# ducha-aiki/mods

Hardware: AMD Instinct MI355X
Metric: image-pairs/sec (1024x768, HessAff+RootSIFT over the affine view ladder, MFMA FGINN match, LO-RANSAC H) (higher is better)
Workload: dtype f32 (detect/describe) + u8 on the int8 matrix cores (distance matrix)

## Files before the change

mods_amd/__init__.py:

```python
import ctypes as C
import os
import subprocess

import numpy as np

_HERE = os.path.dirname(os.path.abspath(__file__))
LIB_PATH = os.environ.get("MODSX_LIB", os.path.join(_HERE, "libmodsx.so"))

KEYPOINT = np.dtype([("x", "f8"), ("y", "f8"), ("a11", "f8"), ("a12", "f8"), ("a21", "f8"), ("a22", "f8"),
                     ("s", "f8"), ("response", "f8"), ("octave_number", "i4"), ("pyramid_scale", "f8"),
                     ("sub_type", "i4")], align=True)
REGION = np.dtype([("img_id", "i4"), ("img_reproj_id", "i4"), ("id", "i4"), ("parent_id", "i4"), ("type", "i4"),
                   ("det_kp", KEYPOINT), ("reproj_kp", KEYPOINT)], align=True)
SSKP = np.dtype([("octave", "i4"), ("level", "i4"), ("r0", "i4"), ("c0", "i4"), ("r", "i4"), ("c", "i4"),
                 ("type", "i4"), ("pad", "i4"), ("b0", "f4"), ("b1", "f4"), ("b2", "f4"), ("val", "f4"),
                 ("x", "f4"), ("y", "f4"), ("s", "f4"), ("pixelDistance", "f4")], align=True)
TENT = np.dtype([("q", "i4"), ("t0", "i4"), ("tj", "i4"), ("t1", "i4"), ("d1", "f8"), ("d2", "f8"),
                 ("d2by2ndcl", "f8"), ("ratio", "f8")], align=True)


class HessAffParams(C.Structure):
    _fields_ = [("threshold", C.c_float), ("mode", C.c_int), ("reg_number", C.c_int),
                ("rel_threshold", C.c_float), ("rel_reg_number", C.c_float), ("numberOfScales", C.c_int),
                ("initialSigma", C.c_float), ("edgeEigenValueRatio", C.c_double), ("border", C.c_int),
                ("maxIterations", C.c_int), ("convergenceThreshold", C.c_float), ("smmWindowSize", C.c_int),
                ("affInitialSigma", C.c_float), ("doBaumberg", C.c_int), ("detectorType", C.c_int)]


class MserParams(C.Structure):
    _fields_ = [("min_size", C.c_int), ("max_area", C.c_double), ("min_margin", C.c_double), ("relative", C.c_int),
                ("mode", C.c_int), ("reg_number", C.c_int), ("rel_threshold", C.c_float), ("rel_reg_number", C.c_float)]


class PairParams(C.Structure):
    _fields_ = [("det", HessAffParams),
                ("ori_mrSize", C.c_double), ("ori_patchSize", C.c_int), ("ori_maxAngles", C.c_int),
                ("ori_threshold", C.c_double),
                ("desc_mrSize", C.c_double), ("desc_patchSize", C.c_int), ("desc_photoNorm", C.c_int),
                ("desc_type", C.c_int), ("desc_maxBinValue", C.c_double),
                ("match_ratio", C.c_double), ("contradDist", C.c_double), ("nn", C.c_int),
                ("duplicateDist", C.c_double),
                ("err_threshold", C.c_double), ("confidence", C.c_double), ("max_samples", C.c_int),
                ("localOptimization", C.c_int), ("HLAFCoef", C.c_double), ("doSymmCheck", C.c_int),
                ("ransac_seed", C.c_uint), ("useF", C.c_int), ("LAFCoef", C.c_double), ("errorType", C.c_int),
                ("detector", C.c_int), ("mser", MserParams),
                ("n_desc", C.c_int), ("desc_types", C.c_int * 4), ("desc_ratios", C.c_double * 4)]


class View(C.Structure):
    _fields_ = [("zoom", C.c_double), ("tilt", C.c_double), ("phi", C.c_double), ("InitSigma", C.c_double),
                ("doBlur", C.c_int)]


def make_view(tilt=1.0, phi=0.0, zoom=1.0, init_sigma=0.5, do_blur=1):
    v = View()
    v.zoom, v.tilt, v.phi, v.InitSigma, v.doBlur = zoom, tilt, phi, init_sigma, do_blur
    return v


def _view_array(views):
    arr = (View * len(views))()
    for i, v in enumerate(views):
        arr[i].zoom, arr[i].tilt, arr[i].phi, arr[i].InitSigma, arr[i].doBlur = v.zoom, v.tilt, v.phi, v.InitSigma, v.doBlur
    return arr


class LadderStep(C.Structure):
    _fields_ = [("views", C.c_void_p), ("nviews", C.c_int), ("match_ratio", C.c_double), ("detector", C.c_int),
                ("n_desc", C.c_int), ("desc_types", C.c_int * 4), ("desc_ratios", C.c_double * 4)]


class PairResult(C.Structure):
    _fields_ = [("n_regions1", C.c_int), ("n_regions2", C.c_int), ("n_tentatives", C.c_int), ("n_unique", C.c_int),
                ("n_ransac_inliers", C.c_int), ("n_verified", C.c_int), ("ransac_samples", C.c_int),
                ("ransac_lo", C.c_int), ("H", C.c_double * 9), ("tentatives", C.c_void_p),
                ("ransac_inlier", C.c_void_p), ("verified", C.c_void_p)]


EXPORTS = ["modsx_version", "modsx_last_error", "modsx_free", "modsx_create", "modsx_destroy", "modsx_synchronize",
           "modsx_default_hessaff_params", "modsx_default_pair_params", "modsx_image_upload", "modsx_image_update",
           "modsx_image_wrap_device", "modsx_image_free", "modsx_image_download", "modsx_detect_affine_keypoints",
           "modsx_detect_scalespace", "modsx_octave_levels", "modsx_gaussian_blur", "modsx_resize_half", "modsx_response",
           "modsx_detect_affine_regions", "modsx_detect_orientation", "modsx_reproject_regions", "modsx_reproject_regions_touch_boundary",
           "modsx_describe_regions", "modsx_match_fginn", "modsx_duplicate_filtering", "modsx_ransac_h",
           "modsx_loransac_h", "modsx_ransac_h_errtype", "modsx_loransac_h_errtype", "modsx_ransac_f", "modsx_loransac_f", "modsx_match_pair", "modsx_match_pairs", "modsx_match_pairs_views", "modsx_pair_result_release",
           "modsx_set_vs_pars", "modsx_synth_view", "modsx_detect_describe_views", "modsx_match_fginn_device",
           "modsx_match_pair_views", "modsx_match_ladder", "modsx_save_regions", "modsx_load_regions", "modsx_default_mser_params", "modsx_detect_msers", "modsx_detect_msers_u8", "modsx_last_timings", "modsx_profile",
           "modsx_kernel_stats", "modsx_last_batch_verify", "modsx_comm_unique_id", "modsx_comm_create", "modsx_comm_destroy", "modsx_comm_info",
           "modsx_view_block_order", "modsx_detect_describe_views_sharded", "modsx_match_fginn_sharded",
           "modsx_match_pair_views_sharded", "modsx_match_pairs_views_sharded", "modsx_match_ladder_sharded", "modsx_comm_loopback_id", "modsx_comm_set_lanes",
           "modsx_comm_attach", "modsx_comm_lane_done", "modsx_comm_reset_lanes", "modsx_comm_set_timeout", "modsx_comm_stats",
           "modsx_shard_block_bytes", "modsx_shard_block_pack", "modsx_shard_blocks_unpack", "modsx_shard_device_pack",
           "modsx_shard_device_unpack", "modsx_verify_device_stats", "modsx_verify_device_timing", "modsx_comm_set_exchange",
           "modsx_shard_owner_plan", "modsx_db_create", "modsx_db_free", "modsx_db_rows", "modsx_db_nearest",
           "modsx_match_fginn_db", "modsx_match_fginn_db_device", "modsx_set_fginn_db"]
EXPORTS_DEGENSAC = ["exp_ransacHcustom", "exp_ransacFcustom", "HDs", "HDsi", "HDsidx", "HDsSym", "HDsiSym", "HDsSymidx",
                    "HDsSymMax", "HDsiSymMax", "HDsSymidxMax", "FDs", "FDsSym", "exFDs", "exFDsSym",
                    "modsx_ransac_set_seed"]

SHARD_ROW_REGION, SHARD_ROW_KP = 0, 1
EXCHANGE_ALL_GATHER, EXCHANGE_OWNER = 0, 1
KP_FIELDS = ("x", "y", "a11", "a12", "a21", "a22", "s")
KERNEL_CLASSES = ["blur_hess", "hessian", "resize", "nms_localize", "baumberg", "orientation", "patch_sample",
                  "blur_rows", "describe", "match_fginn", "gray", "warp_affine", "view_blur", "blur_cols", "match_sweep1", "match_db"]


def build(force=False):
    src = os.path.join(_HERE, "csrc")
    srcs = [os.path.join(src, f) for f in os.listdir(src) if f.endswith((".hip", ".cpp", ".hpp"))]
    srcs.append(os.path.join(_HERE, "..", "include", "modsx.h"))
    stale = (not os.path.exists(LIB_PATH)) or any(os.path.getmtime(s) > os.path.getmtime(LIB_PATH) for s in srcs)
    if force or stale:
        subprocess.check_call(["make", "-C", src, "-j8"], stdout=subprocess.DEVNULL)
    return LIB_PATH


_lib = None


def lib():
    global _lib
    if _lib is None:
        if not os.path.exists(LIB_PATH):
            raise RuntimeError("libmodsx.so is not built; run __graft_entry__.build() (needs hipcc)")
        L = C.CDLL(LIB_PATH)
        L.modsx_last_error.restype = C.c_char_p
        L.modsx_create.restype = C.c_void_p
        L.modsx_create.argtypes = [C.c_int]
        L.modsx_comm_create.restype = C.c_void_p
        L.modsx_comm_create.argtypes = [C.c_void_p, C.c_void_p, C.c_int, C.c_int]
        L.modsx_comm_destroy.argtypes = [C.c_void_p]
        L.modsx_comm_info.argtypes = [C.c_void_p] + [C.c_void_p] * 5
        L.modsx_comm_loopback_id.argtypes = [C.c_void_p, C.c_int]
        L.modsx_comm_set_lanes.argtypes = [C.c_void_p, C.c_int]
        L.modsx_comm_attach.argtypes = [C.c_void_p, C.c_void_p, C.c_int]
        L.modsx_comm_lane_done.argtypes = [C.c_void_p, C.c_int]
        L.modsx_comm_reset_lanes.argtypes = [C.c_void_p]
        L.modsx_comm_set_timeout.argtypes = [C.c_void_p, C.c_int]
        L.modsx_comm_stats.argtypes = [C.c_void_p, C.c_void_p, C.c_int]
        L.modsx_destroy.argtypes = [C.c_void_p]
        L.modsx_free.argtypes = [C.c_void_p]
        L.modsx_image_upload.restype = C.c_void_p
        L.modsx_image_upload.argtypes = [C.c_void_p, C.c_void_p, C.c_int, C.c_int, C.c_int, C.c_int]
        L.modsx_image_update.argtypes = [C.c_void_p, C.c_void_p, C.c_void_p, C.c_int, C.c_int, C.c_int, C.c_int]
        L.modsx_debug_last_batch_verify_each.argtypes = [C.c_void_p, C.c_int]
        L.modsx_image_wrap_device.restype = C.c_void_p
        L.modsx_image_wrap_device.argtypes = [C.c_void_p, C.c_void_p, C.c_int, C.c_int]
        L.modsx_image_free.argtypes = [C.c_void_p, C.c_void_p]
        L.modsx_db_create.restype = C.c_void_p
        L.modsx_db_create.argtypes = [C.c_void_p, C.c_void_p, C.c_long, C.c_int]
        L.modsx_db_free.restype = None
        L.modsx_db_free.argtypes = [C.c_void_p, C.c_void_p]
        L.modsx_db_rows.restype = C.c_long
        L.modsx_db_rows.argtypes = [C.c_void_p]
        L.modsx_db_nearest.argtypes = [C.c_void_p, C.c_void_p, C.c_void_p, C.c_int, C.c_void_p]
        L.modsx_set_fginn_db.argtypes = [C.c_void_p, C.c_void_p]
        L.modsx_synth_view.restype = C.c_void_p
        L.modsx_synth_view.argtypes = [C.c_void_p, C.c_void_p, C.c_void_p, C.c_void_p, C.c_void_p]
        _lib = L
    return _lib


def _err():
    return lib().modsx_last_error().decode()


def _p(a):
    return a.ctypes.data_as(C.c_void_p)


def _check(rc, what):
    if rc < 0:
        raise RuntimeError("%s failed (%d): %s" % (what, rc, _err()))
    return rc


def default_hessaff_params(**kw):
    p = HessAffParams()
    lib().modsx_default_hessaff_params(C.byref(p))
    for k, v in kw.items():
        setattr(p, k, v)
    return p


def default_mser_params(**kw):
    p = MserParams()
    lib().modsx_default_mser_params(C.byref(p))
# ... 685 lines not shown
```

mods_amd/csrc/engine.hip:

```cpp
#include <atomic>
#include <math.h>
#include <stdio.h>
#include <algorithm>
#include <chrono>
#include <map>
#include <unordered_set>
#include <mutex>
#include <dlfcn.h>
#include <string>
#include "engine_api.hpp"

#ifdef MODSX_DUP_BUILD
namespace mx {
int dup_count(int cls) {
  static const long mask = getenv("MODSX_DUP") ? strtol(getenv("MODSX_DUP"), nullptr, 0) : 0;
  return 1 + (int)((mask >> cls) & 1);
}
}
#endif
namespace mx {

static thread_local std::string g_err;
void set_error(const std::string &s) { g_err = s; }
static std::atomic<int> g_busyContexts{0};
// ... 348 lines not shown
  for (int i = 0; i < MAXB; i++) { c->descF[i].release(); c->descU8[i].release(); c->viewImg[i].release(); for (int k = 0; k < 3; k++) c->descU8x[k][i].release(); }
  for (int d = 0; d < 2; d++) for (int t = 0; t < 4; t++) for (int sd = 0; sd < 2; sd++) c->descCls[d][t][sd].release();
  for (int t = 0; t < 4; t++) c->halfDesc[t].release();
  c->candSort.release(); c->candOut.release();
  PinBuf *pins[] = {&c->hCand, &c->hAff, &c->hOri, &c->hDesc, &c->hMisc, &c->hNms, &c->hMatch, &c->hViewTaps, &c->hViewJobs, &c->hMser};
  for (PinBuf *b : pins) b->release();
  hipFree(c->dSmmMask); hipFree(c->dOriMask); hipFree(c->dOriIdx); hipFree(c->dSiftMask); hipFree(c->dSiftMaskIdx); hipFree(c->dAtan); hipFree(c->dOriBinTab); hipFree(c->dSiftOTab); hipFree(c->dSiftBins);
  hipFree(c->dSiftW);
  for (int i = 0; i < 2; i++) hipEventDestroy(c->descEv[i]);
  c->hDescB.release(); c->hRefs.release();
  hipStreamDestroy(c->stream);
  if (c->hFlag) hipHostFree(c->hFlag);
  delete c;
}

static int cv_round(double v) { return (int)lrint(v); }

struct SigmaPlan {
  int levels;
  float sigmaStep;
  float curSigma[8];
  float incSigma[8];
};

static SigmaPlan make_sigma_plan(const modsx_hessaff_params &p) {
  SigmaPlan s;
  s.levels = p.numberOfScales + 2;
  s.sigmaStep = powf(2.0f, 1.0f / (float)p.numberOfScales);
  float cur = p.initialSigma;
  s.curSigma[0] = cur; s.incSigma[0] = 0;
  for (int i = 1; i < s.levels; i++) {
    s.incSigma[i] = cur * sqrtf(s.sigmaStep * s.sigmaStep - 1.0f);
    cur *= s.sigmaStep;
    s.curSigma[i] = cur;
  }
  return s;
}

static int fill_taps(BlurBatch &b, float sigma) {
  int n = blur_ksize(sigma);
  if (n > MAX_TAPS) { set_error("pyramid blur kernel larger than 17 taps is not supported"); return MODSX_ERR_ARG; }
  std::vector<float> k = gaussian_kernel(n, sigma);
  b.n = n;
  for (int i = 0; i < n; i++) b.k[i] = k[i];
  return MODSX_OK;
}

int build_pyramids(modsx_ctx *c, const modsx_image *const *imgs, int n, const modsx_hessaff_params &p,
                   bool singleOctaveFromFirstLevel) {
  if (n <= 0 || n > MAXB) { set_error("batch size"); return MODSX_ERR_ARG; }
  if (p.numberOfScales < 1 || p.numberOfScales > 6) { set_error("numberOfScales"); return MODSX_ERR_ARG; }
  if (p.detectorType != MODSX_DET_HESSIAN && p.detectorType != MODSX_DET_DOG && p.detectorType != MODSX_DET_HARRIS) {
    set_error("detectorType must be Hessian (0), DoG (1) or Harris (2)");
    return MODSX_ERR_ARG;
  }
  const bool hess = p.detectorType == MODSX_DET_HESSIAN;
  const SigmaPlan sp = make_sigma_plan(p);
  const int L = sp.levels;
  const int minSize = 2 * p.border + 2;
  int maxOct = 0;
  for (int i = 0; i < n; i++) {
    Pyramid &py = c->pyr[i];
    py.nOct = 0;
    int rows = imgs[i]->rows, cols = imgs[i]->cols;
    float pd = 1.0f;
    size_t total = 0;
    while (rows > minSize && cols > minSize && py.nOct < 24) {
      Octave &o = py.oct[py.nOct++];
      o.rows = rows; o.cols = cols; o.pixelDistance = pd;
      total += (size_t)2 * L * rows * cols;
      pd *= 2.0;
      rows = cv_round(rows * 0.5); cols = cv_round(cols * 0.5);
      if (singleOctaveFromFirstLevel) break;
    }
    if (!py.store.ensure(total * sizeof(float) + 64)) return MODSX_ERR_NOMEM;
    float *ptr = (float *)py.store.p;
    for (int o = 0; o < py.nOct; o++) {
      size_t npx = (size_t)py.oct[o].rows * py.oct[o].cols;
      for (int l = 0; l < L; l++) { py.oct[o].blur[l] = ptr; ptr += npx; }
      for (int l = 0; l < L; l++) { py.oct[o].resp[l] = ptr; ptr += npx; }
    }
    maxOct = std::max(maxOct, py.nOct);
  }
  hipStream_t s = c->stream;
  for (int o = 0; o < maxOct; o++) {
    BlurBatch bb;
    memset(&bb, 0, sizeof bb);
    int nj = 0, mr = 0, mc = 0;
    if (o == 0) {
      const float curSigma0 = 0.5f;
      const bool preBlur = !singleOctaveFromFirstLevel && p.initialSigma > curSigma0;
      if (preBlur) {
        float sigma = sqrtf(p.initialSigma * p.initialSigma - curSigma0 * curSigma0);
        int rc = fill_taps(bb, sigma);
        if (rc) return rc;
      }
      for (int i = 0; i < n; i++) {
        if (c->pyr[i].nOct <= 0) continue;
        Octave &oc = c->pyr[i].oct[0];
        BlurJob &j = bb.j[nj++];
        j.src = imgs[i]->d; j.blur = oc.blur[0]; j.resp = hess ? oc.resp[0] : nullptr; j.rows = oc.rows; j.cols = oc.cols;
        j.norm = sp.curSigma[0] * sp.curSigma[0];
        mr = std::max(mr, oc.rows); mc = std::max(mc, oc.cols);
        if (!preBlur) {
          MX_HIP(hipMemcpyAsync(oc.blur[0], imgs[i]->d, (size_t)oc.rows * oc.cols * 4, hipMemcpyDeviceToDevice, s));
          j.src = oc.blur[0];
        }
      }
      double px = 0;
      for (int q = 0; q < nj; q++) px += (double)bb.j[q].rows * bb.j[q].cols;
      if (nj) {
        if (preBlur) { ProfScope ps(c, K_BLUR_HESS, px * 12); launch_blur_hess(s, bb, nj, mr, mc); }
        else if (hess) { ProfScope ps(c, K_HESSIAN, px * 8); launch_hessian(s, bb, nj, mr, mc); }
      }
    } else {
      ResizeBatch rb;
      memset(&rb, 0, sizeof rb);
      for (int i = 0; i < n; i++) {
        if (c->pyr[i].nOct <= o) continue;
        Octave &pv = c->pyr[i].oct[o - 1], &oc = c->pyr[i].oct[o];
        ResizeJob &r = rb.j[nj];
        r.src = pv.blur[p.numberOfScales]; r.dst = oc.blur[0];
        r.srows = pv.rows; r.scols = pv.cols; r.drows = oc.rows; r.dcols = oc.cols;
        r.resp = hess ? oc.resp[0] : nullptr; r.norm = sp.curSigma[0] * sp.curSigma[0];
        BlurJob &j = bb.j[nj++];
        j.src = oc.blur[0]; j.blur = nullptr; j.resp = oc.resp[0]; j.rows = oc.rows; j.cols = oc.cols;
        j.norm = sp.curSigma[0] * sp.curSigma[0];
        mr = std::max(mr, oc.rows); mc = std::max(mc, oc.cols);
      }
      if (nj) {
        double spx = 0, dpx = 0;
        for (int q = 0; q < nj; q++) { spx += (double)rb.j[q].srows * rb.j[q].scols; dpx += (double)rb.j[q].drows * rb.j[q].dcols; }
        { ProfScope ps(c, K_RESIZE, (spx + dpx) * 4 + dpx * 4); launch_resize_half(s, rb, nj, mr, mc); }
      }
    }
    if (!nj) continue;
    for (int l = 1; l < L; l++) {
      BlurBatch b2;
      memset(&b2, 0, sizeof b2);
      int rc = fill_taps(b2, sp.incSigma[l]);
      if (rc) return rc;
      int k = 0;
      for (int i = 0; i < n; i++) {
        if (c->pyr[i].nOct <= o) continue;
        Octave &oc = c->pyr[i].oct[o];
        BlurJob &j = b2.j[k++];
        j.src = oc.blur[l - 1]; j.blur = oc.blur[l]; j.resp = hess ? oc.resp[l] : nullptr; j.rows = oc.rows; j.cols = oc.cols;
        j.norm = sp.curSigma[l] * sp.curSigma[l];
      }
      double px = 0;
      for (int q = 0; q < k; q++) px += (double)b2.j[q].rows * b2.j[q].cols;
      ProfScope ps(c, K_BLUR_HESS, px * 12);
      launch_blur_hess(s, b2, k, mr, mc);
    }
    if (!hess) {
      for (int l = 0; l < L; l++) {
        const float norm = sp.curSigma[l] * sp.curSigma[l];
        const float sigma = p.detectorType == MODSX_DET_DOG ? norm : sqrtf((float)(0.6 * norm));
        const int nt = blur_ksize(sigma);
        if (2 * nt > 2 * 4096) { set_error("response blur kernel too large"); return MODSX_ERR_ARG; }
        if (!c->viewTaps.ensure((size_t)L * 2 * 4100 * 4) || !c->hViewTaps.ensure((size_t)L * 2 * 4100 * 4)) return MODSX_ERR_NOMEM;
        float *dT = (float *)c->viewTaps.p + (size_t)l * 2 * 4100, *hT = (float *)c->hViewTaps.p + (size_t)l * 2 * 4100;
        bool tapsUp = false;
        for (int i = 0; i < n; i++) {
          if (c->pyr[i].nOct <= o) continue;
          Octave &oc = c->pyr[i].oct[o];
          const int rows = oc.rows, cols = oc.cols;
          const size_t npx = (size_t)rows * cols;
          if (!c->scratchA.ensure(npx * 4 * 8)) return MODSX_ERR_NOMEM;
          float *buf = (float *)c->scratchA.p, *tmp = buf, *a = buf + npx, *b = buf + 2 * npx, *cc = buf + 3 * npx;
          float *ba = buf + 4 * npx, *bb2 = buf + 5 * npx, *bc = buf + 6 * npx;
          const int nx = cols == 1 ? 1 : nt, ny = rows == 1 ? 1 : nt;
          if (!tapsUp || nx != nt || ny != nt) {
            std::vector<float> kx = gaussian_kernel(nx, sigma), ky = gaussian_kernel(ny, sigma);
            if (tapsUp) MX_HIP(ctx_sync(c));
            memcpy(hT, kx.data(), nx * 4); memcpy(hT + nx, ky.data(), ny * 4);
            MX_HIP(ctx_copy(c, dT, hT, (size_t)(nx + ny) * 4, hipMemcpyHostToDevice));
            tapsUp = nx == nt && ny == nt;
          }
          auto blur = [&](const float *src, float *dst) {
            if (nt == 1) { MX_HIP(hipMemcpyAsync(dst, src, npx * 4, hipMemcpyDeviceToDevice, s)); return MODSX_OK; }
            launch_blur_pass(s, src, tmp, rows, cols, dT, nx, 0, 1);
            launch_blur_pass(s, tmp, dst, rows, cols, dT + nx, ny, 1, 1);
            return MODSX_OK;
          };
          if (p.detectorType == MODSX_DET_DOG) {
            int rc = blur(oc.blur[l], a);
            if (rc) return rc;
            launch_sub(s, oc.blur[l], a, oc.resp[l], npx);
          } else {
            launch_grad_products(s, oc.blur[l], rows, cols, a, b, cc);
            int rc = blur(a, ba);
            if (!rc) rc = blur(b, bb2);
            if (!rc) rc = blur(cc, bc);
            if (rc) return rc;
            launch_harris_combine(s, ba, bb2, bc, (float)(0.6 * norm), oc.resp[l], npx);
          }
        }
      }
    }
  }
  MX_HIP(hipGetLastError());
  return MODSX_OK;
}

static const unsigned CAND_CAP = 1u << 21;

int detect_scalespace_batch(modsx_ctx *c, const modsx_image *const *imgs, int n, const modsx_hessaff_params &p,
                            std::vector<modsx_sskp> *out) {
  int rc = build_pyramids(c, imgs, n, p, false);
  if (rc) return rc;
  hipStream_t s = c->stream;
  if (!c->cand.ensure((size_t)CAND_CAP * sizeof(Candidate)) || !c->nmsQueue.ensure((size_t)CAND_CAP * 16)) return MODSX_ERR_NOMEM;
  if (!c->counter.ensure((NMS_QUEUES + 1) * 128)) return MODSX_ERR_NOMEM;
  MX_HIP(hipMemsetAsync(c->counter.p, 0, 128 + NMS_QUEUES * 128, s));
  bool queuesClean = true;
  NmsBatch nb;
  memset(&nb, 0, sizeof nb);
  nb.edgeScoreThreshold = (p.edgeEigenValueRatio + 1.0f) * (p.edgeEigenValueRatio + 1.0f) / p.edgeEigenValueRatio;
  float finalTh = p.threshold;
  float posTh = (float)(0.8 * finalTh);
  float negTh = -posTh;
  if (p.detectorType == MODSX_DET_HESSIAN) finalTh = p.threshold * p.threshold;
  if (p.mode != MODSX_FIXED_TH) finalTh = posTh = negTh = 0.0f;
  nb.posTh = posTh; nb.negTh = negTh; nb.finalTh = finalTh; nb.border = p.border; nb.detType = p.detectorType;
  int maxOct = 0;
  for (int i = 0; i < n; i++) maxOct = std::max(maxOct, c->pyr[i].nOct);
  const bool perOctave = p.numberOfScales == 3 && !getenv("MODSX_NMS_PER_LEVEL");
  std::vector<NmsJob> hjobs;
  std::vector<int> hpfx(1, 0), hfirst;
  double px = 0;
  auto flush = [&](bool last) -> int {
    const int nj = (int)hjobs.size();
    if (!nj) return MODSX_OK;
    const int np = (int)hpfx.size() - 1;
    const size_t jobBytes = (size_t)nj * sizeof(NmsJob), pfxBytes = (size_t)(np + 1) * 4, firstBytes = (size_t)std::max<size_t>(1, hfirst.size()) * 4;
    if (!c->nmsJobs.ensure(jobBytes + pfxBytes + firstBytes + 64)) return MODSX_ERR_NOMEM;
    if (!c->hNms.ensure(jobBytes + pfxBytes + firstBytes)) return MODSX_ERR_NOMEM;
    memcpy(c->hNms.p, hjobs.data(), jobBytes);
    memcpy((char *)c->hNms.p + jobBytes, hpfx.data(), pfxBytes);
    if (!hfirst.empty()) memcpy((char *)c->hNms.p + jobBytes + pfxBytes, hfirst.data(), hfirst.size() * 4);
    MX_HIP(ctx_copy(c, c->nmsJobs.p, c->hNms.p, jobBytes + pfxBytes + firstBytes, hipMemcpyHostToDevice));
    if (!c->tileJob.ensure((size_t)hpfx.back() * 4 + 4)) return MODSX_ERR_NOMEM;
    const int *dPfx = (const int *)((char *)c->nmsJobs.p + jobBytes);
    launch_expand_tiles(s, dPfx, np, (int *)c->tileJob.p);
    {
      ProfScope ps(c, K_NMS, px * 12);
      if (!queuesClean) MX_HIP(hipMemsetAsync((unsigned *)c->counter.p + 32, 0, NMS_QUEUES * 128, s));
      queuesClean = false;
      launch_nms(s, nb, (const NmsJob *)c->nmsJobs.p, dPfx, (const int *)c->tileJob.p, nj,
                 hpfx.back(), (int4 *)c->nmsQueue.p, (unsigned *)c->counter.p + 32, CAND_CAP, (Candidate *)c->cand.p,
                 (unsigned *)c->counter.p, CAND_CAP, perOctave ? (const int *)((char *)c->nmsJobs.p + jobBytes + pfxBytes) : nullptr,
                 p.numberOfScales);
    }
    if (!last) MX_HIP(ctx_sync(c));
    hjobs.clear(); hpfx.assign(1, 0); hfirst.clear(); px = 0;
    return MODSX_OK;
  };
  for (int o = 0; o < maxOct; o++)
    for (int i = 0; i < n; i++) {
      if (c->pyr[i].nOct <= o) continue;
      Octave &oc = c->pyr[i].oct[o];
      const int w = oc.cols - 2 * p.border, h = oc.rows - 2 * p.border;
      if (w <= 0 || h <= 0) continue;
      if ((int)hjobs.size() + p.numberOfScales > NMS_MAXJ) { int rcf = flush(false); if (rcf) return rcf; }
      const int tiles = ((w + 63) / 64) * ((h + NMS_TILE_ROWS - 1) / NMS_TILE_ROWS);
      if (perOctave) { hfirst.push_back((int)hjobs.size()); hpfx.push_back(hpfx.back() + tiles); }
      for (int l = 1; l <= p.numberOfScales; l++) {
        NmsJob j;
        j.low = oc.resp[l - 1]; j.cur = oc.resp[l]; j.high = oc.resp[l + 1]; j.blur = oc.blur[l];
        j.rows = oc.rows; j.cols = oc.cols; j.img = i; j.octave = o; j.level = l; j.pad = 0;
        hjobs.push_back(j);
        if (!perOctave) hpfx.push_back(hpfx.back() + tiles);
        px += (double)oc.rows * oc.cols;
      }
    }
  { int rcf = flush(true); if (rcf) return rcf; }
  static const bool deviceOrder = getenv("MODSX_DEVICE_ORDER") != nullptr && atoi(getenv("MODSX_DEVICE_ORDER")) != 0;
  if (deviceOrder) {
    typedef size_t (*temp_fn)(unsigned);
    typedef int (*order_fn)(hipStream_t, const Candidate *, const unsigned *, unsigned, unsigned long long *, unsigned long long *, unsigned *, unsigned *,
                            void *, size_t, unsigned long long *, unsigned *, unsigned, unsigned *, Candidate *, unsigned *);
// ... 1205 lines not shown
```

mods_amd/csrc/engine.hpp:

```cpp
#pragma once
#include <hip/hip_runtime.h>
#include <stdint.h>
#include <stdlib.h>
#include <string.h>
#include <string>
#include <vector>
#include "../../include/modsx.h"
#include "kmath.hpp"

namespace mx {

#ifndef MODSX_MAXB
#define MODSX_MAXB 32
#endif
constexpr int MAXB = MODSX_MAXB;
constexpr int PAIR_GROUP = 4;
constexpr int NMS_MAXJ = 1024;
constexpr int MAX_TAPS = 17;

struct BlurJob {
  const float *src;
  float *blur;
  float *resp;
  int rows, cols;
  float norm;
  int pad;
};
struct BlurBatch {
  int n;
  float k[MAX_TAPS];
  BlurJob j[MAXB];
  int nj;
  int tile0[MAXB + 1];
};
struct ResizeJob {
  const float *src;
  float *dst;
  float *resp;
  int srows, scols, drows, dcols;
  float norm;
  int pad;
};
struct ResizeBatch { ResizeJob j[MAXB]; int nj; int tile0[MAXB + 1]; };
struct NmsJob {
  const float *low, *cur, *high, *blur;
  int rows, cols, img, octave, level, pad;
};
struct NmsBatch {
  float posTh, negTh, finalTh;
  int border;
  double edgeScoreThreshold;
  int detType, pad;
};
struct Candidate {
  int img, octave, level, type;
  int r0, c0, r, c;
  float b0, b1, b2, val;
};

struct AffJob {
  const float *blur;
  int rows, cols;
  float x, y, s, pixelDistance;
};
struct AffOut { float u11, u12, u21, u22; int ok; int iters; };

struct OriJob {
  int img;
  float x, y, a11, a12, a21, a22;
};
constexpr int ORI_MAX_PEAKS = 18;

struct DescJob {
  int img;
  int P;
  int ksize;
  int tapOfs;
  float x, y, a11, a12, a21, a22;
  float i2p;
  int NC;
  int needOfs;
  int coordOfs;
  int touch;
  int outIdx;
  int rows0;
  int ro1;
  unsigned long long scratchOfs;
  unsigned long long rowOfs;
  unsigned long long gridOfs;
};
struct BlurTile {
  unsigned long long srcOfs, dstOfs;
  int P, NC, n, tapOfs, needOfs;
  int job, pad;
  int first, count, lo, span, magic;
};
struct ImgRef { const float *d; int rows, cols, pad; };
struct DescOut { float *f[MAXB]; uint8_t *u8[MAXB]; uint8_t *u8x[3][MAXB]; };

struct WarpJob {
  const float *src;
  float *dst;
  int srows, scols, drows, dcols;
  double M[6];
  float cval;
  int pad;
};

struct ViewJob {
  const float *src;
  float *rot, *tmp, *dst;
  int srows, scols, rrows, rcols, drows, dcols;
  int kx, ky, tapOfs, doBlur;
  int tileA, tileB;
  int tileF, fused;
  int tileG, pad;
  double R[6], W[6];
  double invW[2];
};

struct MatchRow {
  int t0, t1, nless, nbad;
  int tj;
  float dj;
  float d0, d1;
};
static_assert(sizeof(MatchRow) == 32, "match rows are 32 bytes");

struct DevBuf {
  void *p = nullptr;
  size_t cap = 0;
  bool ensure(size_t bytes);
  void release();
};
struct PinBuf {
  void *p = nullptr;
  size_t cap = 0;
  bool ensure(size_t bytes);
  void release();
};

struct Octave {
  int rows, cols;
  float pixelDistance;
  float *blur[8];
  float *resp[8];
};
struct Pyramid {
  int nOct = 0;
  Octave oct[24];
  DevBuf store;
};

void set_error(const std::string &s);
bool gpu_shared();
struct CtxBusy { modsx_ctx *c; explicit CtxBusy(modsx_ctx *c); ~CtxBusy(); CtxBusy(const CtxBusy &) = delete; CtxBusy &operator=(const CtxBusy &) = delete; };
hipError_t ctx_copy(modsx_ctx *c, void *dst, const void *src, size_t bytes, hipMemcpyKind kind);
hipError_t ctx_sync(modsx_ctx *c);
unsigned ctx_mark(modsx_ctx *c);
bool ctx_mark_reached(modsx_ctx *c, unsigned seq);
hipError_t ctx_wait_mark(modsx_ctx *c, unsigned seq);
bool host_wait_runtime();
int host_cpus_per_rank();
#define MX_HIP(expr)                                                                          \
  do {                                                                                        \
    hipError_t e_ = (expr);                                                                   \
    if (e_ != hipSuccess) {                                                                   \
      mx::set_error(std::string(#expr) + ": " + hipGetErrorString(e_));                       \
      return MODSX_ERR_DEVICE;                                                                \
    }                                                                                         \
  } while (0)

std::vector<float> gaussian_kernel(int n, double sigma);
int blur_ksize(float sigma);
void gauss_mask(float *mask, int size);
void circular_gauss_mask(float *mask, int size, float sigma);
const double *atan_lut_host();
inline bool check_borders_host(int w, int h, float ofsx, float ofsy, float a11, float a12, float a21, float a22, int rw, int rh) {
  return check_borders(w, h, ofsx, ofsy, a11, a12, a21, a22, rw, rh);
}
bool invert3(const double *S, double *t);
void rectify(double &a11, double &a12, double &a21, double &a22);

void launch_blur_hess(hipStream_t s, const BlurBatch &b, int nj, int maxRows, int maxCols);
void launch_hessian(hipStream_t s, const BlurBatch &b, int nj, int maxRows, int maxCols);
void launch_resize_half(hipStream_t s, const ResizeBatch &b, int nj, int maxRows, int maxCols);
void launch_nms(hipStream_t s, const NmsBatch &b, const NmsJob *jobs, const int *tilePrefix, const int *tileJob, int nj,
                int nTiles, int4 *queue, unsigned *qcount, unsigned qcap, Candidate *out, unsigned *counter, unsigned cap,
                const int *octFirst = nullptr, int levelsPerOctave = 0);
size_t cand_sort_temp_bytes(unsigned nsort);
int launch_cand_order(hipStream_t s, const Candidate *cand, const unsigned *counter, unsigned nsort, unsigned long long *keys,
                      unsigned long long *keys2, unsigned *idx, unsigned *idx2, void *temp, size_t tempBytes, unsigned long long *tabKey,
                      unsigned *tabRank, unsigned tabSize, unsigned *slotOf, Candidate *out, unsigned *outCount);
constexpr int NMS_QUEUES = 64;
constexpr int NMS_TILE_ROWS = 16;
void launch_gray(hipStream_t s, const void *src, float *dst, size_t n, int channels, int dtype);
void launch_baumberg(hipStream_t s, const AffJob *jobs, AffOut *out, int n, const float *mask, int W, int maxIter,
                     float convTh, float affInitialSigma);
constexpr int ATAN_CASES = 2048 + 64;
constexpr int ORI_NV = 1344;
void launch_orientation(hipStream_t s, const OriJob *jobs, float *out, int n, const ImgRef *imgs,
                        const unsigned short *maskIdx, const float *maskW,
                        const unsigned char *binTab, int doHalf, double th, int maxAngles);
void launch_trunc_u8(hipStream_t s, const float *src, uint8_t *dst, size_t n);
size_t mser_sort_blocks(const int *rows, int n);
void launch_mser_sort(hipStream_t s, const uint8_t *const *u8, const int *rows, const int *cols, const size_t *ordOfs, int n, int *blockHist,
                      int *start, int *order);
void launch_expand_blur_tiles(hipStream_t s, const DescJob *jobs, const int *prefixRows, const int *prefixCols, int nJobs,
                              const int *needTab, BlurTile *tilesRows, BlurTile *tilesCols, float2 *rowStarts);
void launch_sample_rows(hipStream_t s, const DescJob *jobs, const BlurTile *tiles, int nTiles, const ImgRef *imgs, const float *taps,
                        const int *needTab, float *dst, const float2 *rowStarts, float *dstGrid);
void launch_blur_cols(hipStream_t s, const BlurTile *tiles, int nTiles, const float *taps, const int *needTab, const float *src,
                      float *dst);
void launch_expand_tiles(hipStream_t s, const int *prefix, int nJobs, int *tileJob);
void launch_patch_sample(hipStream_t s, const DescJob *jobs, const int *tilePrefix, const int *tileJob, int nTiles,
                         const ImgRef *imgs, float *scratch);
void launch_patch_blur(hipStream_t s, const DescJob *jobs, const int *tilePrefix, const int *tileJob, int nTiles,
                       const float *taps, const int *needTab, const float *src, float *dst, int pass);
void launch_describe(hipStream_t s, const DescJob *jobs, int n, const ImgRef *imgs, const float *grid,
                     const int *needTab, const float *coordTab,
                     const float *mask, const unsigned short *maskIdx, int nmask, const float *oTab, const int *bins,
                     const double *wts, int photoNorm, int descTypes, int nOut, double maxBin, const DescOut &outs);
void launch_warp_affine(hipStream_t s, const WarpJob &jb);
void launch_blur_pass(hipStream_t s, const float *src, float *dst, int rows, int cols, const float *taps, int n, int pass, int border = 0);
void launch_sub(hipStream_t s, const float *a, const float *b, float *o, size_t n);
void launch_grad_products(hipStream_t s, const float *img, int rows, int cols, float *xx, float *yy, float *xy);
void launch_harris_combine(hipStream_t s, const float *bxx, const float *byy, const float *bxy, float sigmasq, float *o, size_t n);
void launch_views_warp(hipStream_t s, const ViewJob *jobs, int n, int tiles, int stage);
void launch_views_blur(hipStream_t s, const ViewJob *jobs, int n, int tiles, const float *taps, int pass);
constexpr int VF_TW = 128, VF_TH = 16, VF_RX = 32, VF_RY = 2;
void launch_views_rotblur(hipStream_t s, const ViewJob *jobs, int n, int tiles, const float *taps, int maxRx, int maxRy);
void launch_views_fused(hipStream_t s, const ViewJob *jobs, int n, int tiles, const float *taps, int maxRx, int maxRy);
size_t match_workspace_bytes(int n1, int n2);
void launch_match(hipStream_t s, const uint8_t *d1, int n1, const uint8_t *d2, int n2, const double *pos2,
                  double sqminratio, double contrDistSq, int nn, MatchRow *rows, void *workspace);
#ifndef MODSX_SR_WIN
#define MODSX_SR_WIN 2400
#define MODSX_FC_ROWS 40
#define MODSX_SR_HALF 1
#define MODSX_SR_WGS 8
#endif
#ifndef MODSX_BLUR_LDS_C
#define MODSX_BLUR_LDS_C 9984
#endif
constexpr int MATCH_NN_MAX = 256;
constexpr int MATCH_MAXB = 4;
void launch_match_batch(hipStream_t s, int nb, const uint8_t *const *d1, const int *n1, const uint8_t *const *d2, const int *n2,
                        const double *const *pos2, double sqminratio, double contrDistSq, int nn, MatchRow *const *rows,
                        void *const *workspace, hipEvent_t *evSweep1 = nullptr);
struct DbGeo { int TEp, TOp; };
struct DbSet {
  DevBuf store;
  const unsigned char *tiles = nullptr;
  const int *hrow = nullptr;
  DbGeo geo = {0, 0};
  long rows = 0;
  int dev = 0;
};
DbGeo db_geo(long n, long nOdd);
size_t db_tiles_bytes(const DbGeo &g);
size_t db_hrow_bytes(const DbGeo &g);
int db_pack_blocks(long n);
void launch_db_pack(hipStream_t s, const uint8_t *raw, long n, const int2 *base, long nOdd, const DbGeo &geo, unsigned char *tiles,
                    int *hrow);
void launch_db_select(hipStream_t s, int nb, const MatchRow *const *rows, const int *n1, int nn, bool allPoints, int *const *sel, int *cnt,
                      int *const *dmin);
void launch_dbnn_min(hipStream_t s, int nb, const uint8_t *const *d1, const int *n1, int *const *sel, int *cnt, int *const *dmin,
                     const DbSet &db);

}

namespace mx {
#ifdef MODSX_DUP_BUILD
int dup_count(int cls);
#define MX_DUP(cls) for (int dupLeft_ = mx::dup_count(cls); dupLeft_ > 0; dupLeft_--)
#else
#define MX_DUP(cls)
#endif
enum KClass { K_BLUR_HESS = 0, K_HESSIAN, K_RESIZE, K_NMS, K_BAUMBERG, K_ORIENT, K_PATCH_SAMPLE, K_BLUR_ROWS, K_DESCRIBE,
              K_MATCH, K_GRAY, K_WARP, K_VIEW_BLUR, K_BLUR_COLS, K_MATCH_SWEEP1, K_MATCH_DB, K_NCLASS };
struct Profiler {
  bool enabled = false;
  std::vector<hipEvent_t> evA, evB;
  std::vector<int> cls;
  size_t used = 0;
  double ms[K_NCLASS] = {0};
  double work[K_NCLASS] = {0};
  long launches[K_NCLASS] = {0};
};
}

struct modsx_db { mx::DbSet set; };

struct modsx_image {
  float *d;
  int rows, cols;
  bool owned;
};

struct modsx_ctx {
  int dev;
  hipStream_t stream;
  mx::Pyramid pyr[mx::MAXB];
  mx::DevBuf candSort, candOut;
  size_t lastSurvivors = 0;
  mx::DevBuf nmsJobs, cand, counter, affJobs, affOut, oriJobs, oriOut, descJobs, tilePrefix, taps, imgRefs, scratchA, scratchB,
      descF[mx::MAXB], descU8[mx::MAXB], descAllF[2], descAllU8[2], descAllU8b[2], descCls[2][4][2], descU8x[3][mx::MAXB], shardLocal, pos2, matchRows, matchWork, dbSel, misc, viewTmp[2], viewTaps, viewJobs, viewImg[mx::MAXB], scratchC, needTab, coordTab, tileJob, blurTiles, nmsQueue, rowStarts;
  mx::ImgRef imgRefsHost[mx::MAXB];
  mx::PinBuf hDescB;
  hipEvent_t descEv[2];
  bool descEvPending[2] = {false, false};
  bool descByEvent[2] = {true, true};
  unsigned descMark[2] = {0, 0};
  unsigned *hFlag = nullptr;
  unsigned flagSeq = 0;
  bool waitRuntime = true;
  mx::PinBuf hCand, hAff, hOri, hDesc, hMisc, hNms, hMatch, hViewTaps, hViewJobs, hMser, hRefs;
  float *dSmmMask = nullptr;
  int smmW = 0;
  std::vector<uint64_t> candKeys, candKeys2, candClaim;
  std::vector<uint32_t> candOrder, candOrder2;
  float *dOriMask = nullptr;
  unsigned short *dOriIdx = nullptr;
  float *dSiftMask = nullptr;
  unsigned short *dSiftMaskIdx = nullptr;
  int nSiftMask = 0;
  double *dAtan = nullptr;
  unsigned char *dOriBinTab = nullptr;
  float *dSiftOTab = nullptr;
  int *dSiftBins = nullptr;
  double *dSiftW = nullptr;
  double timings[6];
  mx::Profiler prof;
  size_t lastCandCount = 0;
  const mx::DbSet *fginnDb = nullptr;
  int busyDepth = 0;
  int shardLane = 0;
  modsx_ctx *peer = nullptr;
  modsx_ctx *half = nullptr;
  mx::DevBuf halfDesc[4];
  void *worker = nullptr;
};
```

mods_amd/csrc/kernels_pyramid.hip:

```cpp
#include "engine.hpp"

namespace mx {

constexpr int TW = 64;
constexpr int TMP_W = TW + 4;

MX_D int find_job(const int *tile0, int nj, int t) {
  int j = 0;
  while (j + 1 < nj && t >= tile0[j + 1]) j++;
  return j;
}

typedef float f2 __attribute__((ext_vector_type(2)));

template <int R, int TH>
__global__ __launch_bounds__(256) void k_blur_hess(BlurBatch batch) {
  constexpr int BLR_H = TH + 4;
  const int ji = find_job(batch.tile0, batch.nj, blockIdx.x);
  const BlurJob jb = batch.j[ji];
  const int rows = jb.rows, cols = jb.cols;
  const int lt = blockIdx.x - batch.tile0[ji], ntx = (cols + TW - 1) / TW;
  const int tx0 = (lt % ntx) * TW, ty0 = (lt / ntx) * TH;
  constexpr int n = 2 * R + 1;
  constexpr int sh = BLR_H + 2 * R, sw = TMP_W + 2 * R;
// ... 76 lines not shown
      if (gy >= 1 && gy < rows - 1 && gx >= 1 && gx < cols - 1) {
        const float v11 = B[-TMP_W - 1], v12 = B[-TMP_W], v13 = B[-TMP_W + 1];
        const float v21 = B[-1], v22 = B[0], v23 = B[1];
        const float v31 = B[TMP_W - 1], v32 = B[TMP_W], v33 = B[TMP_W + 1];
        float Lxx = (v21 - 2 * v22 + v23);
        float Lyy = (v12 - 2 * v22 + v32);
        float Lxy = (v13 - v11 + v31 - v33) / 4.0f;
        o = (Lxx * Lyy - Lxy * Lxy) * norm2;
      }
      jb.resp[gofs] = o;
    }
  }
}

__global__ __launch_bounds__(256) void k_hessian(BlurBatch batch) {
  const int ji = find_job(batch.tile0, batch.nj, blockIdx.x);
  const BlurJob jb = batch.j[ji];
  const int rows = jb.rows, cols = jb.cols;
  const int lt = blockIdx.x - batch.tile0[ji], ntx = (cols + 63) / 64;
  const int gx = (lt % ntx) * 64 + (threadIdx.x & 63), gy = (lt / ntx) * 4 + (threadIdx.x >> 6);
  if (gx >= cols || gy >= rows) return;
  float o = 0.f;
  if (gy >= 1 && gy < rows - 1 && gx >= 1 && gx < cols - 1) {
    const float *B = jb.src + (size_t)gy * cols + gx;
    const float v11 = B[-cols - 1], v12 = B[-cols], v13 = B[-cols + 1];
    const float v21 = B[-1], v22 = B[0], v23 = B[1];
    const float v31 = B[cols - 1], v32 = B[cols], v33 = B[cols + 1];
    float Lxx = (v21 - 2 * v22 + v23);
    float Lyy = (v12 - 2 * v22 + v32);
    float Lxy = (v13 - v11 + v31 - v33) / 4.0f;
    o = (Lxx * Lyy - Lxy * Lxy) * (jb.norm * jb.norm);
  }
  jb.resp[(size_t)gy * cols + gx] = o;
}

MX_D float resize_half_px(const float *src, int sr, int sc, int dx, int dy) {
  const int sy0 = dy * 2, sx0 = dx * 2;
  float out;
  if (sy0 >= sr) out = 0.f;
  else if (sy0 + 2 <= sr && dx < sc / 2) {
    const float *S = src + (size_t)sy0 * sc + sx0;
    float sum = 0.f;
    sum = sum + (((S[0] + S[1]) + S[sc]) + S[sc + 1]);
    out = sum * 0.25f;
  } else {
    float sum = 0.f; int count = 0;
    for (int sy = 0; sy < 2; sy++) {
      if (sy0 + sy >= sr) break;
      for (int sx = 0; sx < 2; sx++) {
        if (sx0 + sx >= sc) break;
        sum += src[(size_t)(sy0 + sy) * sc + sx0 + sx];
        count++;
      }
    }
    out = (sx0 >= sc) ? 0.f : sum / (float)count;
  }
  return out;
}
__global__ __launch_bounds__(256) void k_resize_half(ResizeBatch batch) {
  const int ji = find_job(batch.tile0, batch.nj, blockIdx.x);
  const ResizeJob jb = batch.j[ji];
  const int lt = blockIdx.x - batch.tile0[ji], ntx = (jb.dcols + 63) / 64;
  const int dx = (lt % ntx) * 64 + (threadIdx.x & 63), dy = (lt / ntx) * 4 + (threadIdx.x >> 6);
  if (dx >= jb.dcols || dy >= jb.drows) return;
  const int sr = jb.srows, sc = jb.scols, rows = jb.drows, cols = jb.dcols;
  const float v22 = resize_half_px(jb.src, sr, sc, dx, dy);
  jb.dst[(size_t)dy * cols + dx] = v22;
  if (!jb.resp) return;
  float o = 0.f;
  if (dy >= 1 && dy < rows - 1 && dx >= 1 && dx < cols - 1) {
    const float v11 = resize_half_px(jb.src, sr, sc, dx - 1, dy - 1), v12 = resize_half_px(jb.src, sr, sc, dx, dy - 1),
                v13 = resize_half_px(jb.src, sr, sc, dx + 1, dy - 1);
    const float v21 = resize_half_px(jb.src, sr, sc, dx - 1, dy), v23 = resize_half_px(jb.src, sr, sc, dx + 1, dy);
    const float v31 = resize_half_px(jb.src, sr, sc, dx - 1, dy + 1), v32 = resize_half_px(jb.src, sr, sc, dx, dy + 1),
                v33 = resize_half_px(jb.src, sr, sc, dx + 1, dy + 1);
    float Lxx = (v21 - 2 * v22 + v23);
    float Lyy = (v12 - 2 * v22 + v32);
    float Lxy = (v13 - v11 + v31 - v33) / 4.0f;
    o = (Lxx * Lyy - Lxy * Lxy) * (jb.norm * jb.norm);
  }
  jb.resp[(size_t)dy * cols + dx] = o;
}

MX_D bool is_max9(float val, const float *p, int cols) {
  bool ok = true;
#pragma unroll
  for (int dr = -1; dr <= 1; dr++)
#pragma unroll
    for (int dc = -1; dc <= 1; dc++) ok = ok && !(p[dr * cols + dc] > val);
  return ok;
}
MX_D bool is_min9(float val, const float *p, int cols) {
  bool ok = true;
#pragma unroll
  for (int dr = -1; dr <= 1; dr++)
#pragma unroll
    for (int dc = -1; dc <= 1; dc++) ok = ok && !(p[dr * cols + dc] < val);
  return ok;
}

constexpr int NMS_ROWS = 16, NMS_LW = 66, NMS_REFINE_BLOCKS = 16;

MX_D bool nms_refine(const NmsBatch &batch, const NmsJob &jb, int r, int c, Candidate &k) {
  const int rows = jb.rows, cols = jb.cols;
  const int r0 = r, c0 = c;
  float b[3] = {0.f, 0.f, 0.f};
  float val = 0.f;
  int nr = r, nc = c;
  for (int iter = 0; iter < 5; iter++) {
    r = nr; c = nc;
    const float *c1 = jb.cur + (size_t)r * cols, *c0p = c1 - cols, *c2 = c1 + cols;
    const float *l1 = jb.low + (size_t)r * cols, *l0 = l1 - cols, *l2 = l1 + cols;
    const float *h1 = jb.high + (size_t)r * cols, *h0 = h1 - cols, *h2 = h1 + cols;
    float dxx = c1[c - 1] - 2.0f * c1[c] + c1[c + 1];
    float dyy = c0p[c] - 2.0f * c1[c] + c2[c];
    float dss = l1[c] - 2.0f * c1[c] + h1[c];
    float dxy = 0.25f * (c2[c + 1] - c2[c - 1] - c0p[c + 1] + c0p[c - 1]);
    if (iter == 0) {
      float edgeScore = (dxx + dyy) * (dxx + dyy) / (dxx * dyy - dxy * dxy);
      if ((double)edgeScore >= batch.edgeScoreThreshold || edgeScore < 0) return false;
    }
    float dxs = 0.25f * (h1[c + 1] - h1[c - 1] - l1[c + 1] + l1[c - 1]);
    float dys = 0.25f * (h2[c] - h0[c] - l2[c] + l0[c]);
    float A[9] = {dxx, dxy, dxs, dxy, dyy, dys, dxs, dys, dss};
    float dx = 0.5f * (c1[c + 1] - c1[c - 1]);
    float dy = 0.5f * (c2[c] - c0p[c]);
    float ds = 0.5f * (h1[c] - l1[c]);
    b[0] = -dx; b[1] = -dy; b[2] = -ds;
    solve3(A, b);
    if (isnan(b[0]) || isnan(b[1]) || isnan(b[2])) return false;
    val = c1[c] + 0.5f * (dx * b[0] + dy * b[1] + ds * b[2]);
    if ((double)b[0] > 0.6) { if (c < cols - 3) nc++; else return false; }
    if ((double)b[1] > 0.6) { if (r < rows - 3) nr++; else return false; }
    if ((double)b[0] < -0.6) { if (c > 3) nc--; else return false; }
    if ((double)b[1] < -0.6) { if (r > 3) nr--; else return false; }
    if (nr == r && nc == c) break;
  }
  if (fabsf(b[0]) > 1.5f || fabsf(b[1]) > 1.5f || fabsf(b[2]) > 1.5f || fabsf(val) < batch.finalTh) return false;
  int type;
  if (batch.detType == MODSX_DET_DOG) type = val < 0 ? 11 : 10;
  else if (batch.detType == MODSX_DET_HARRIS) type = val < 0 ? 31 : 30;
  else if (val < 0) type = 2;
  else {
    const float *p = jb.blur + (size_t)r * cols + c;
    float Lxx = (p[-1] - 2 * p[0] + p[1]);
    type = (Lxx < 0) ? 0 : 1;
  }
  k.img = jb.img; k.octave = jb.octave; k.level = jb.level; k.type = type;
  k.r0 = r0; k.c0 = c0; k.r = r; k.c = c;
  k.b0 = b[0]; k.b1 = b[1]; k.b2 = b[2]; k.val = val;
  return true;
}

__global__ __launch_bounds__(256) void k_nms_localize(NmsBatch batch, const NmsJob *__restrict__ jobs,
                                                      const int *__restrict__ tilePrefix, const int *__restrict__ tileJob,
                                                      int4 *queue, unsigned *qcount, unsigned qcap, unsigned *overflow) {
  const int tile = blockIdx.x;
  const int jid = tileJob[tile];
  const NmsJob jb = jobs[jid];
  const int rows = jb.rows, cols = jb.cols, B = batch.border;
  const int local = tile - tilePrefix[jid];
  const int tilesX = (cols - 2 * B + 63) / 64;
  const int by = local / tilesX, bx = local - by * tilesX;
  const int r0 = B + by * NMS_ROWS, c0 = B + bx * 64;
  __shared__ float sp[3][NMS_ROWS + 2][NMS_LW];
  {
// ... 385 lines not shown
```

Before: 217.5.

## Fuse small pyramid octaves into one LDS-resident kernel per image

For octaves below a pixel threshold, the resize, all per-level separable blurs and the Hessian response are now computed in a single kernel. Each image gets one 1024-thread block that holds the working planes in LDS, replacing many tiny per-level launches. This removes launch overhead and global round-trips on small octaves. The cost is low parallelism, one block per image, and a large LDS footprint, and the fused path must reproduce the existing resize and border semantics exactly.

```diff
diff --git a/mods_amd/__init__.py b/mods_amd/__init__.py
--- a/mods_amd/__init__.py
+++ b/mods_amd/__init__.py
@@ -102,7 +102,8 @@
 EXCHANGE_ALL_GATHER, EXCHANGE_OWNER = 0, 1
 KP_FIELDS = ("x", "y", "a11", "a12", "a21", "a22", "s")
 KERNEL_CLASSES = ["blur_hess", "hessian", "resize", "nms_localize", "baumberg", "orientation", "patch_sample",
-                  "blur_rows", "describe", "match_fginn", "gray", "warp_affine", "view_blur", "blur_cols", "match_sweep1", "match_db"]
+                  "blur_rows", "describe", "match_fginn", "gray", "warp_affine", "view_blur", "blur_cols", "match_sweep1", "match_db",
+                  "pyr_small"]
 
 
 def build(force=False):
diff --git a/mods_amd/csrc/engine.hip b/mods_amd/csrc/engine.hip
--- a/mods_amd/csrc/engine.hip
+++ b/mods_amd/csrc/engine.hip
@@ -454,6 +454,20 @@
     }
     maxOct = std::max(maxOct, py.nOct);
   }
+  int lim[MAXB];
+  for (int i = 0; i < n; i++) lim[i] = c->pyr[i].nOct;
+  {
+    const char *e = getenv("MODSX_PYR_SMALL_OCTAVES");
+    bool small = hess && !singleOctaveFromFirstLevel && !(e && !atoi(e)) && L <= PYR_SMALL_MAXL;
+    for (int l = 1; small && l < L; l++) { const int nt = blur_ksize(sp.incSigma[l]); small = nt >= 3 && nt <= MAX_TAPS; }
+    for (int i = 0; small && i < n; i++) {
+      const Pyramid &py = c->pyr[i];
+      for (int o = 1; o < py.nOct; o++)
+        if ((long)py.oct[o].rows * pyr_small_stride(py.oct[o].cols) <= PYR_SMALL_PX) { lim[i] = o; break; }
+      for (int o = lim[i]; o < py.nOct; o++)
+        if (py.oct[o].rows != pyr_half_dim(py.oct[o - 1].rows) || py.oct[o].cols != pyr_half_dim(py.oct[o - 1].cols)) lim[i] = py.nOct;
+    }
+  }
   hipStream_t s = c->stream;
   for (int o = 0; o < maxOct; o++) {
     BlurBatch bb;
@@ -489,7 +503,7 @@
       ResizeBatch rb;
       memset(&rb, 0, sizeof rb);
       for (int i = 0; i < n; i++) {
-        if (c->pyr[i].nOct <= o) continue;
+        if (lim[i] <= o) continue;
         Octave &pv = c->pyr[i].oct[o - 1], &oc = c->pyr[i].oct[o];
         ResizeJob &r = rb.j[nj];
         r.src = pv.blur[p.numberOfScales]; r.dst = oc.blur[0];
@@ -514,7 +528,7 @@
       if (rc) return rc;
       int k = 0;
       for (int i = 0; i < n; i++) {
-        if (c->pyr[i].nOct <= o) continue;
+        if (lim[i] <= o) continue;
         Octave &oc = c->pyr[i].oct[o];
         BlurJob &j = b2.j[k++];
         j.src = oc.blur[l - 1]; j.blur = oc.blur[l]; j.resp = hess ? oc.resp[l] : nullptr; j.rows = oc.rows; j.cols = oc.cols;
@@ -570,6 +584,34 @@
           }
         }
       }
+    }
+  }
+  {
+    PyrSmallBatch pb;
+    memset(&pb, 0, sizeof pb);
+    pb.L = L;
+    double bytes = 0;
+    for (int i = 0; i < n; i++) {
+      Pyramid &py = c->pyr[i];
+      if (lim[i] >= py.nOct) continue;
+      const Octave &pv = py.oct[lim[i] - 1];
+      PyrSmallJob &j = pb.j[pb.nj++];
+      j.seed = pv.blur[p.numberOfScales]; j.srows = pv.rows; j.scols = pv.cols;
+      j.dst = py.oct[lim[i]].blur[0]; j.nOct = py.nOct - lim[i];
+      bytes += (double)pv.rows * pv.cols * 4;
+      for (int o = lim[i]; o < py.nOct; o++) bytes += (double)2 * L * py.oct[o].rows * py.oct[o].cols * 4;
+    }
+    if (pb.nj) {
+      for (int l = 0; l < L; l++) pb.norm[l] = sp.curSigma[l] * sp.curSigma[l];
+      for (int l = 1; l < L; l++) {
+        BlurBatch t;
+        int rc = fill_taps(t, sp.incSigma[l]);
+        if (rc) return rc;
+        pb.n[l] = t.n;
+        for (int q = 0; q < t.n; q++) pb.k[l][q] = t.k[q];
+      }
+      ProfScope ps(c, K_PYR_SMALL, bytes);
+      launch_pyr_small(s, pb);
     }
   }
   MX_HIP(hipGetLastError());
diff --git a/mods_amd/csrc/engine.hpp b/mods_amd/csrc/engine.hpp
--- a/mods_amd/csrc/engine.hpp
+++ b/mods_amd/csrc/engine.hpp
@@ -42,6 +42,26 @@
   int pad;
 };
 struct ResizeBatch { ResizeJob j[MAXB]; int nj; int tile0[MAXB + 1]; };
+#ifndef MODSX_PYR_SMALL_PX
+#define MODSX_PYR_SMALL_PX 12288
+#endif
+constexpr int PYR_SMALL_PX = MODSX_PYR_SMALL_PX;
+constexpr int PYR_SMALL_MAXL = 8;
+inline int pyr_small_stride(int cols) { return (cols + 3) & ~3; }
+MX_HD int pyr_half_dim(int v) { const int h = v >> 1; return (v & 1) ? h + (h & 1) : h; }
+struct PyrSmallJob {
+  const float *seed;
+  float *dst;
+  int srows, scols;
+  int nOct, pad;
+};
+struct PyrSmallBatch {
+  PyrSmallJob j[MAXB];
+  int nj, L;
+  int n[PYR_SMALL_MAXL];
+  float k[PYR_SMALL_MAXL][MAX_TAPS];
+  float norm[PYR_SMALL_MAXL];
+};
 struct NmsJob {
   const float *low, *cur, *high, *blur;
   int rows, cols, img, octave, level, pad;
@@ -185,6 +205,7 @@
 void launch_blur_hess(hipStream_t s, const BlurBatch &b, int nj, int maxRows, int maxCols);
 void launch_hessian(hipStream_t s, const BlurBatch &b, int nj, int maxRows, int maxCols);
 void launch_resize_half(hipStream_t s, const ResizeBatch &b, int nj, int maxRows, int maxCols);
+void launch_pyr_small(hipStream_t s, const PyrSmallBatch &b);
 void launch_nms(hipStream_t s, const NmsBatch &b, const NmsJob *jobs, const int *tilePrefix, const int *tileJob, int nj,
                 int nTiles, int4 *queue, unsigned *qcount, unsigned qcap, Candidate *out, unsigned *counter, unsigned cap,
                 const int *octFirst = nullptr, int levelsPerOctave = 0);
@@ -278,7 +299,7 @@
 #define MX_DUP(cls)
 #endif
 enum KClass { K_BLUR_HESS = 0, K_HESSIAN, K_RESIZE, K_NMS, K_BAUMBERG, K_ORIENT, K_PATCH_SAMPLE, K_BLUR_ROWS, K_DESCRIBE,
-              K_MATCH, K_GRAY, K_WARP, K_VIEW_BLUR, K_BLUR_COLS, K_MATCH_SWEEP1, K_MATCH_DB, K_NCLASS };
+              K_MATCH, K_GRAY, K_WARP, K_VIEW_BLUR, K_BLUR_COLS, K_MATCH_SWEEP1, K_MATCH_DB, K_PYR_SMALL, K_NCLASS };
 struct Profiler {
   bool enabled = false;
   std::vector<hipEvent_t> evA, evB;
diff --git a/mods_amd/csrc/kernels_pyramid.hip b/mods_amd/csrc/kernels_pyramid.hip
--- a/mods_amd/csrc/kernels_pyramid.hip
+++ b/mods_amd/csrc/kernels_pyramid.hip
@@ -182,6 +182,176 @@
   jb.resp[(size_t)dy * cols + dx] = o;
 }
 
+#ifndef MODSX_PS_THREADS
+#define MODSX_PS_THREADS 1024
+#endif
+constexpr int PS_THREADS = MODSX_PS_THREADS;
+
+template <typename P>
+MX_D float resize_half_px_st(P src, int st, int sr, int sc, int dx, int dy) {
+  const int sy0 = dy * 2, sx0 = dx * 2;
+  float out;
+  if (sy0 >= sr) out = 0.f;
+  else if (sy0 + 2 <= sr && dx < sc / 2) {
+    const int b = sy0 * st + sx0;
+    float sum = 0.f;
+    sum = sum + (((src[b] + src[b + 1]) + src[b + st]) + src[b + st + 1]);
+    out = sum * 0.25f;
+  } else {
+    float sum = 0.f; int count = 0;
+    for (int sy = 0; sy < 2; sy++) {
+      if (sy0 + sy >= sr) break;
+      for (int sx = 0; sx < 2; sx++) {
+        if (sx0 + sx >= sc) break;
+        sum += src[(sy0 + sy) * st + sx0 + sx];
+        count++;
+      }
+    }
+    out = (sx0 >= sc) ? 0.f : sum / (float)count;
+  }
+  return out;
+}
+
+struct PsDiv { unsigned d, m; };
+MX_D PsDiv ps_div_of(int d) { return PsDiv{(unsigned)d, 0xffffffffu / (unsigned)d + 1u}; }
+MX_D int ps_div(int i, PsDiv q) { return q.d == 1u ? i : (int)__umulhi((unsigned)i, q.m); }
+
+template <int R>
+MX_D void ps_blur(const float *cur, float *tmp, float *nxt, int rows, int cols, int st, const float *kk, PsDiv dc, PsDiv dg) {
+  constexpr int n = 2 * R + 1;
+  constexpr int H = (R + 3) / 4;
+  float k[n];
+#pragma unroll
+  for (int j = 0; j < n; j++) k[j] = kk[j];
+  const int tid = threadIdx.x;
+  const int ng = st >> 2;
+  for (int i = tid; i < rows * ng; i += PS_THREADS) {
+    const int y = ps_div(i, dg), x0 = 4 * (i - y * ng);
+    const float *S = cur + y * st;
+    float w[4 * (2 * H + 1)];
+#pragma unroll
+    for (int d = 0; d <= 2 * H; d++) {
+      const int cx = x0 + 4 * (d - H);
+      if (cx >= 0 && cx + 3 < cols) {
+        const float4 t = *reinterpret_cast<const float4 *>(S + cx);
+        w[4 * d] = t.x; w[4 * d + 1] = t.y; w[4 * d + 2] = t.z; w[4 * d + 3] = t.w;
+      } else {
+#pragma unroll
+        for (int e = 0; e < 4; e++) {
+          int x = cx + e;
+          x = x < 0 ? 0 : (x > cols - 1 ? cols - 1 : x);
+          w[4 * d + e] = S[x];
+        }
+      }
+    }
+    float v[4];
+#pragma unroll
+    for (int o = 0; o < 4; o++) {
+      constexpr int c0 = 4 * H;
+      if (n <= 5) {
+        v[o] = w[c0 + o] * k[R];
+#pragma unroll
+        for (int j = 1; j <= R; j++) v[o] = v[o] + (w[c0 + o - j] + w[c0 + o + j]) * k[R + j];
+      } else {
+        v[o] = 0.f;
+#pragma unroll
+        for (int j = 0; j < n; j++) v[o] = v[o] + w[c0 + o - R + j] * k[j];
+      }
+    }
+    *reinterpret_cast<float4 *>(tmp + y * st + x0) = make_float4(v[0], v[1], v[2], v[3]);
+  }
+  __syncthreads();
+  const int ng4 = (rows + 3) >> 2;
+  for (int i = tid; i < ng4 * cols; i += PS_THREADS) {
+    const int gy = ps_div(i, dc), x = i - gy * cols, y0 = 4 * gy;
+    float w[4 + 2 * R];
+#pragma unroll
+    for (int q = 0; q < 4 + 2 * R; q++) {
+      int y = y0 - R + q;
+      y = y < 0 ? 0 : (y > rows - 1 ? rows - 1 : y);
+      w[q] = tmp[y * st + x];
+    }
+#pragma unroll
+    for (int o = 0; o < 4; o++) {
+      float v = w[o + R] * k[R] + 0.f;
+#pragma unroll
+      for (int j = 1; j <= R; j++) v = v + (w[o + R + j] + w[o + R - j]) * k[R + j];
+      if (y0 + o < rows) nxt[(y0 + o) * st + x] = v;
+    }
+  }
+  __syncthreads();
+}
+
+MX_D void ps_emit(const float *pl, int rows, int cols, int st, float norm, float *blur, float *resp, PsDiv dc) {
+  const float norm2 = norm * norm;
+  for (int i = threadIdx.x; i < rows * cols; i += PS_THREADS) {
+    const int y = ps_div(i, dc), x = i - y * cols;
+    const float *B = pl + y * st + x;
+    blur[i] = B[0];
+    float o = 0.f;
+    if (y >= 1 && y < rows - 1 && x >= 1 && x < cols - 1) {
+      const float v11 = B[-st - 1], v12 = B[-st], v13 = B[-st + 1];
+      const float v21 = B[-1], v22 = B[0], v23 = B[1];
+      const float v31 = B[st - 1], v32 = B[st], v33 = B[st + 1];
+      float Lxx = (v21 - 2 * v22 + v23);
+      float Lyy = (v12 - 2 * v22 + v32);
+      float Lxy = (v13 - v11 + v31 - v33) / 4.0f;
+      o = (Lxx * Lyy - Lxy * Lxy) * norm2;
+    }
+    resp[i] = o;
+  }
+}
+
+__global__ __launch_bounds__(PS_THREADS) void k_pyr_small(PyrSmallBatch batch) {
+  __shared__ __attribute__((aligned(16))) float lds[3 * PYR_SMALL_PX];
+  const PyrSmallJob jb = batch.j[blockIdx.x];
+  const int L = batch.L;
+  int cur = 0, tmp = PYR_SMALL_PX, nxt = 2 * PYR_SMALL_PX;
+  int sr = jb.srows, sc = jb.scols, sst = 0;
+  float *out = jb.dst;
+  for (int oi = 0; oi < jb.nOct; oi++) {
+    const int rows = pyr_half_dim(sr), cols = pyr_half_dim(sc), st = (cols + 3) & ~3;
+    if (rows * st > PYR_SMALL_PX) break;
+    const int npx = rows * cols;
+    const PsDiv dc = ps_div_of(cols), dg = ps_div_of(st >> 2);
+    if (oi == 0) {
+      const auto src = as_global(jb.seed);
+      for (int i = threadIdx.x; i < npx; i += PS_THREADS) {
+        const int y = ps_div(i, dc), x = i - y * cols;
+        lds[tmp + y * st + x] = resize_half_px_st(src, sc, sr, sc, x, y);
+      }
+    } else {
+      for (int i = threadIdx.x; i < npx; i += PS_THREADS) {
+        const int y = ps_div(i, dc), x = i - y * cols;
+        lds[tmp + y * st + x] = resize_half_px_st(lds + nxt, sst, sr, sc, x, y);
+      }
+    }
+    __syncthreads();
+    { const int t = cur; cur = tmp; tmp = t; }
+    ps_emit(lds + cur, rows, cols, st, batch.norm[0], out, out + (size_t)L * npx, dc);
+    for (int l = 1; l < L; l++) {
+      const float *kk = batch.k[l];
+      switch (batch.n[l] >> 1) {
+        case 1: ps_blur<1>(lds + cur, lds + tmp, lds + nxt, rows, cols, st, kk, dc, dg); break;
+        case 2: ps_blur<2>(lds + cur, lds + tmp, lds + nxt, rows, cols, st, kk, dc, dg); break;
+        case 3: ps_blur<3>(lds + cur, lds + tmp, lds + nxt, rows, cols, st, kk, dc, dg); break;
+        case 4: ps_blur<4>(lds + cur, lds + tmp, lds + nxt, rows, cols, st, kk, dc, dg); break;
+        case 5: ps_blur<5>(lds + cur, lds + tmp, lds + nxt, rows, cols, st, kk, dc, dg); break;
+        case 6: ps_blur<6>(lds + cur, lds + tmp, lds + nxt, rows, cols, st, kk, dc, dg); break;
+        case 7: ps_blur<7>(lds + cur, lds + tmp, lds + nxt, rows, cols, st, kk, dc, dg); break;
+        default: ps_blur<8>(lds + cur, lds + tmp, lds + nxt, rows, cols, st, kk, dc, dg); break;
+      }
+      { const int t = cur; cur = nxt; nxt = t; }
+      ps_emit(lds + cur, rows, cols, st, batch.norm[l], out + (size_t)l * npx, out + (size_t)(L + l) * npx, dc);
+    }
+    out += (size_t)2 * L * npx;
+    sr = rows; sc = cols; sst = st;
+  }
+}
+void launch_pyr_small(hipStream_t s, const PyrSmallBatch &b) {
+  if (b.nj > 0) MX_DUP(K_PYR_SMALL) hipLaunchKernelGGL(k_pyr_small, dim3(b.nj), dim3(PS_THREADS), 0, s, b);
+}
+
 MX_D bool is_max9(float val, const float *p, int cols) {
   bool ok = true;
 #pragma unroll
```

After: 218.4 (median of 2 runs). No clear change (+0.4%).
